# lebrice/blurred-GAN

Measured on AMD Instinct MI355X. Metric: images/sec (G+D+GP step), higher is better.
Workload: dtype f32; 1 GPU; celeba64 64x64x3 batch 256/GPU, blur sigma 5.0 (31 taps), D-step+GP+G-step+Adam; global_batch=256, parallelism=dp1

## Files before the change

### blurred-gan_amd/csrc/conv_wgrad.hip

```cpp
#include "conv_common.h"
#include <algorithm>
#include <cmath>
#include <cstdlib>
#include <mutex>
#include <type_traits>
#include <utility>

namespace {

typedef float floatx16 __attribute__((ext_vector_type(16)));

struct WgradParams {
  const float* X;
  const float* DY;
  float* out;
  int B, H, W, Ci, Ho, Wo, Co;
  int k, s, pt, pl;
  int M;
  int chunk;
  int ksplit;
  int tiles_m, tiles_n, xcd_swizzle;
  float beta, scale;
  unsigned x_bytes, dy_bytes;
  unsigned mul_hw, sh_hw, mul_w, sh_w;
// ... 988 lines not shown
    }
  };

  int strip = blockIdx.x;
  prefetch(strip);
  stash(0);
  __syncthreads();
  int buf = 0;
  for (; strip < nstrips; strip += gridDim.x, buf ^= 1) {
#pragma unroll
    for (int ks = 0; ks < KSW; ++ks) { bc[ks][0] = bn[ks][0]; bc[ks][1] = bn[ks][1]; }
    prefetch(strip + gridDim.x);
    const float* xb = c16_lds + buf * kC16Rows * RS + (2 * r) * RS + (half * (WO / 2) + kq + 1) * 16 + li;
#pragma unroll
    for (int ks = 0; ks < KSW; ++ks)
#pragma unroll
      for (int kh = 0; kh < 5; ++kh)
#pragma unroll
        for (int kw = 0; kw < 5; ++kw) {
          const int par = (kw + 1) & 1, fl = kw == 0 ? -1 : (kw - 1) / 2;
          const float a = xb[kh * RS + par * PS + (4 * ks + fl) * 16];
          acc[kh * 5 + kw][0] = __builtin_amdgcn_mfma_f32_16x16x4f32(a, bc[ks][0], acc[kh * 5 + kw][0], 0, 0, 0);
          acc[kh * 5 + kw][1] = __builtin_amdgcn_mfma_f32_16x16x4f32(a, bc[ks][1], acc[kh * 5 + kw][1], 0, 0, 0);
        }
    stash(buf ^ 1);
    __syncthreads();
  }
  float* red = c16_lds;
  for (int w = 0; w < 4; ++w) {
    __syncthreads();
    if (wave == w) {
#pragma unroll
      for (int t = 0; t < 25; ++t)
#pragma unroll
        for (int nt = 0; nt < 2; ++nt)
#pragma unroll
          for (int rr = 0; rr < 4; ++rr) {
            float* q = red + ((t * 2 + nt) * 4 + rr) * 64 + lane;
            *q = (w == 0 ? 0.f : *q) + acc[t][nt][rr];
          }
    }
  }
  __syncthreads();
  float* out = p.out + (size_t)blockIdx.x * 25 * 16 * 32;
  for (int e = tid; e < 25 * 2 * 4 * 64; e += 256) {
    const int l = e & 63, slot = e >> 6;
    const int rr = slot & 3, nt = (slot >> 2) & 1, t = slot >> 3;
    out[(size_t)(t * 16 + 4 * (l >> 4) + rr) * 32 + nt * 16 + (l & 15)] = red[e];
  }
}

template <int LGWO>
struct StripGeom {
  static constexpr int WO = 1 << LGWO, W = 2 * WO, R = 64 / WO, RX = 2 * R + 3, WP = W + 3;
  static constexpr int XROW = WP * 32, XBUF = RX * XROW, YBUF = 64 * 64, BUF = XBUF + YBUF;
  static constexpr int NX = RX * W * 8, NLX = (NX + 255) / 256, NL = NLX + 4;
  static constexpr size_t lds_bytes = (size_t)2 * BUF * sizeof(float);
};

typedef float floatx2 __attribute__((ext_vector_type(2)));

template <int O0>
__device__ inline void strip_read2(floatx2& dst, unsigned addr) {
  asm volatile("ds_read2st64_b32 %0, %1 offset0:%2 offset1:%3" : "=v"(dst) : "v"(addr), "n"(O0), "n"(O0 + 2));
}
__device__ inline void strip_mfma(floatx16& acc, float a, float b) {
  asm volatile("v_mfma_f32_32x32x2_f32 %0, %1, %2, %0" : "+a"(acc) : "v"(a), "v"(b));
}
template <int LGWO, int Q, int T>
__device__ inline void strip_fetch(floatx2 (&af)[13], floatx2& bf, const unsigned (&aaddr)[13], unsigned baddr) {
  constexpr int WO = 1 << LGWO, WP = 2 * WO + 3, pix = 4 * Q, oyl = pix >> LGWO, ox = pix & (WO - 1);
  if constexpr (T < 13) strip_read2<oyl * WP + ox>(af[T], aaddr[T]);
  else strip_read2<pix>(bf, baddr);
}
typedef float floatx4v __attribute__((ext_vector_type(4)));
__device__ inline void strip_gload(floatx4v& dst, unsigned off, __amdgpu_buffer_rsrc_t rs) {
  asm volatile("buffer_load_dwordx4 %0, %1, %2, 0 offen" : "=v"(dst) : "v"(off), "s"(rs));
}
template <int VM>
__device__ inline void strip_lwrite(unsigned addr, const floatx4v& v) {
  asm volatile("s_waitcnt vmcnt(%2)\n\tds_write_b128 %0, %1" : : "v"(addr), "v"(v), "n"(VM) : "memory");
}
template <int NL_, int PPP_>
struct StripPieces {
  static constexpr int NL = NL_, PPP = PPP_, LAG = 3;
  floatx4v pf[NL_];
  unsigned off[NL_];
  unsigned dst[NL_];
  __amdgpu_buffer_rsrc_t rsX, rsY;
  int nlx;
};
template <int LGWO, int Q, int I, class PC>
__device__ inline void strip_steps(floatx16 (&acc)[13], floatx2 (&af)[2][13], floatx2 (&bf)[2], const unsigned (&aaddr)[13], unsigned baddr,
                                   bool mine, PC& pc) {
  if constexpr (I < 26) {
    constexpr int C = Q & 1, H = I / 13, T = I % 13;
    if (T < 12 || mine) {
      if constexpr (H == 0) strip_mfma(acc[T], af[C][T].x, bf[C].x);
      else strip_mfma(acc[T], af[C][T].y, bf[C].y);
    }
    if constexpr (Q + 1 < 16 && I <= 13) strip_fetch<LGWO, Q + 1, I>(af[C ^ 1], bf[C ^ 1], aaddr, baddr);
    constexpr int P = PC::PPP, NL = PC::NL, LAG = PC::LAG;
    if constexpr (I >= 14 && I <= 18 && ((I - 14) & 1) == 0) {
      constexpr int u = (I - 14) / 2, l = Q * P + u;
      if constexpr (u < P && l < NL) {
        if (l < pc.nlx) strip_gload(pc.pf[l], pc.off[l], pc.rsX);
        else strip_gload(pc.pf[l], pc.off[l], pc.rsY);
      }
    }
    if constexpr (I >= 19 && I <= 23 && ((I - 19) & 1) == 0) {
      constexpr int u = (I - 19) / 2, lw = (Q - LAG) * P + u;
      if constexpr (Q >= LAG && u < P && lw < NL) {
        constexpr int issued = (Q + 1) * P < NL ? (Q + 1) * P : NL;
        strip_lwrite<issued - lw - 1>(pc.dst[lw], pc.pf[lw]);
      }
    }
    strip_steps<LGWO, Q, I + 1>(acc, af, bf, aaddr, baddr, mine, pc);
  }
}
template <int LGWO, int T>
__device__ inline void strip_fetch_first(floatx2 (&af)[2][13], floatx2 (&bf)[2], const unsigned (&aaddr)[13], unsigned baddr) {
  if constexpr (T <= 13) {
    strip_fetch<LGWO, 0, T>(af[0], bf[0], aaddr, baddr);
    strip_fetch_first<LGWO, T + 1>(af, bf, aaddr, baddr);
  }
}
template <int LGWO, int Q, class PC>
__device__ inline void strip_pairs(floatx16 (&acc)[13], floatx2 (&af)[2][13], floatx2 (&bf)[2], const unsigned (&aaddr)[13], unsigned baddr,
                                   PC& pc, int th) {
  if constexpr (Q < 16) {
    asm volatile("s_waitcnt lgkmcnt(0)" ::: "memory");
    strip_steps<LGWO, Q, 0>(acc, af, bf, aaddr, baddr, (Q & 1) == th, pc);
    strip_pairs<LGWO, Q + 1>(acc, af, bf, aaddr, baddr, pc, th);
  }
}

template <int LGWO>
__global__ __launch_bounds__(256, 1) void conv_wgrad_strip_kernel(const WgradParams p, int nstrips, int strips_per_img, int strips_per_wg,
                                                                   int ntile) {
  using G = StripGeom<LGWO>;
  constexpr int WO = G::WO, W = G::W, R = G::R, RX = G::RX, WP = G::WP, XROW = G::XROW, XBUF = G::XBUF, BUF = G::BUF;
  constexpr int NLX = G::NLX, NL = G::NL, NT = 13;
  constexpr unsigned kOob = 0x80000000u;
  extern __shared__ __attribute__((aligned(16))) float strip_lds[];
  const int tid = threadIdx.x, lane = tid & 63, wave = __builtin_amdgcn_readfirstlane(tid >> 6);
  const int th = wave >> 1, nh = wave & 1;
  int tile, z;
  {
    const int idx = blockIdx.x;
    if ((p.ksplit & 7) == 0) {
      const int j = idx >> 3;
      tile = j % ntile;
      z = (idx & 7) + 8 * (j / ntile);
    } else {
      tile = idx % ntile;
      z = idx / ntile;
    }
  }
  const int tile_m = tile / p.tiles_n, tile_n = tile - tile_m * p.tiles_n;
  const int ci0 = tile_m * 32, co0 = tile_n * 64;
  const __amdgpu_buffer_rsrc_t rsX = __builtin_amdgcn_make_buffer_rsrc(const_cast<float*>(p.X), 0, (int)p.x_bytes, 0x00020000);
  const __amdgpu_buffer_rsrc_t rsY = __builtin_amdgcn_make_buffer_rsrc(const_cast<float*>(p.DY), 0, (int)p.dy_bytes, 0x00020000);

  for (int i = tid; i < 2 * RX * 3 * 32; i += 256) {
    const int e = i & 31, rest = i >> 5, c = rest % 3, row = rest / 3;
    const int bufi = row / RX, rr = row - bufi * RX;
    strip_lds[bufi * BUF + rr * XROW + (c == 0 ? 0 : (W + c)) * 32 + e] = 0.f;
  }

  floatx16 acc[NT];
#pragma unroll
  for (int t = 0; t < NT; ++t)
#pragma unroll
    for (int r = 0; r < 16; ++r) acc[t][r] = 0.f;

  constexpr int NP = 16, LAG = 3, PPP = (NL + NP - LAG - 1) / (NP - LAG) > 2 ? (NL + NP - LAG - 1) / (NP - LAG) : 2;
  static_assert(PPP <= 3 && PPP * (NP - LAG) >= NL, "every piece of the next strip must be requested and written within one strip");
  StripPieces<NL, PPP> pc;
  pc.rsX = rsX; pc.rsY = rsY; pc.nlx = NLX;
  int x_rr[NLX], x_dst[NLX];
  unsigned x_off[NLX];
#pragma unroll
  for (int l = 0; l < NLX; ++l) {
    const int item = l * 256 + tid;
    const int rr = item / (W * 8), rem = item - rr * (W * 8);
    const int xc = rem >> 3, q = rem & 7;
    x_rr[l] = item < G::NX ? rr : 1 << 20;
    x_dst[l] = item < G::NX ? rr * XROW + (xc + 1) * 32 + q * 4 : (tid & 7) * 4;
    x_off[l] = (unsigned)(((rr * W + xc) * p.Ci + ci0 + q * 4) * 4);
  }
  const int y_dst = XBUF + (tid >> 4) * 64 + (tid & 15) * 4;
  const unsigned y_off = (unsigned)(((tid >> 4) * p.Co + co0 + (tid & 15) * 4) * 4);

  const int s_begin = z * strips_per_wg, s_end = min(nstrips, s_begin + strips_per_wg);
  auto plan = [&](int sidx, int buf) {
    const bool live = sidx < s_end;
    const int b = sidx / strips_per_img, oy0 = (sidx - b * strips_per_img) * R;
    const unsigned xbase = (unsigned)(((b * p.H + 2 * oy0 - 1) * W) * p.Ci * 4);
    const unsigned ybase = (unsigned)(((b * p.Ho + oy0) * WO) * p.Co * 4);
#pragma unroll
    for (int l = 0; l < NL; ++l) {
      if (l < NLX) {
        const int y = 2 * oy0 - 1 + x_rr[l];
        const bool ok = live && (unsigned)y < (unsigned)p.H;
        pc.off[l] = ok ? xbase + x_off[l] : kOob;
        pc.dst[l] = (unsigned)((buf * BUF + x_dst[l]) * 4);
      } else {
        pc.off[l] = live ? ybase + (unsigned)((l - NLX) * 16 * p.Co * 4) + y_off : kOob;
        pc.dst[l] = (unsigned)((buf * BUF + y_dst + (l - NLX) * 16 * 64) * 4);
      }
    }
  };

  plan(s_begin, 0);
#pragma unroll
  for (int l = 0; l < NL; ++l) {
    if (l < NLX) strip_gload(pc.pf[l], pc.off[l], rsX);
    else strip_gload(pc.pf[l], pc.off[l], rsY);
  }
#pragma unroll
  for (int l = 0; l < NL; ++l) {
    if (l == 0) strip_lwrite<0>(pc.dst[l], pc.pf[l]);
    else asm volatile("ds_write_b128 %0, %1" : : "v"(pc.dst[l]), "v"(pc.pf[l]) : "memory");
  }
  asm volatile("s_waitcnt lgkmcnt(0)" ::: "memory");
  __syncthreads();

  const int kk = lane >> 5, li = lane & 31;
  int a_tap[NT];
#pragma unroll
  for (int t = 0; t < NT; ++t) {
    const int tap = t < 12 ? th * 13 + t : 12;
    const int kh = tap / 5, kw = tap - kh * 5;
    a_tap[t] = (kh * WP + kw) * 32 + kk * 64 + li;
  }
  const int b_base = XBUF + kk * 64 + nh * 32 + li;

  int buf = 0;
  for (int sidx = s_begin; sidx < s_end; ++sidx, buf ^= 1) {
    unsigned aaddr[NT];
#pragma unroll
    for (int t = 0; t < NT; ++t) aaddr[t] = (unsigned)((buf * BUF + a_tap[t]) * 4);
    const unsigned baddr = (unsigned)((buf * BUF + b_base) * 4);
    floatx2 af[2][NT], bf[2];
    plan(sidx + 1, buf ^ 1);
    asm volatile("" ::: "memory");
    strip_fetch_first<LGWO, 0>(af, bf, aaddr, baddr);
    strip_pairs<LGWO, 0>(acc, af, bf, aaddr, baddr, pc, th);
    asm volatile("s_waitcnt lgkmcnt(0)" ::: "memory");
    __syncthreads();
  }

  if (th == 1) {
#pragma unroll
    for (int r = 0; r < 16; ++r) strip_lds[(nh * 16 + r) * 64 + lane] = acc[12][r];
  }
  __syncthreads();
  if (th == 0) {
#pragma unroll
    for (int r = 0; r < 16; ++r) acc[12][r] += strip_lds[(nh * 16 + r) * 64 + lane];
  }
  float* out = p.out + (size_t)z * 25 * p.Ci * p.Co;
#pragma unroll
  for (int t = 0; t < NT; ++t) {
    const int tap = t < 12 ? th * 13 + t : 12;
    if (t < 12 || th == 0) {
      float* o = out + (size_t)tap * p.Ci * p.Co + (size_t)ci0 * p.Co + co0 + nh * 32 + li;
#pragma unroll
      for (int r = 0; r < 16; ++r) o[(size_t)((r & 3) + 8 * (r >> 2) + 4 * kk) * p.Co] = acc[t][r];
    }
  }
}

__global__ __launch_bounds__(256) void wgrad_reduce_kernel(const float* __restrict__ slabs, float* __restrict__ dw, int n,
                                                           int ksplit, float beta, float scale) {
  __shared__ float4 red[4][64];
  const int lane = threadIdx.x & 63, zg = threadIdx.x >> 6;
  const int e = (blockIdx.x * 64 + lane) * 4;
  float4 s = make_float4(0.f, 0.f, 0.f, 0.f);
  if (e < n) {
    int z = zg;
    for (; z + 12 < ksplit; z += 16) {
      float4 v[4];
#pragma unroll
      for (int i = 0; i < 4; ++i) v[i] = *reinterpret_cast<const float4*>(slabs + (size_t)(z + 4 * i) * n + e);
#pragma unroll
      for (int i = 0; i < 4; ++i) { s.x += v[i].x; s.y += v[i].y; s.z += v[i].z; s.w += v[i].w; }
    }
    {
      float4 v[4];
#pragma unroll
      for (int i = 0; i < 4; ++i)
        v[i] = z + 4 * i < ksplit ? *reinterpret_cast<const float4*>(slabs + (size_t)(z + 4 * i) * n + e) : make_float4(0.f, 0.f, 0.f, 0.f);
#pragma unroll
      for (int i = 0; i < 4; ++i)
        if (z + 4 * i < ksplit) { s.x += v[i].x; s.y += v[i].y; s.z += v[i].z; s.w += v[i].w; }
    }
  }
  red[zg][lane] = s;
  __syncthreads();
  if (zg != 0 || e >= n) return;
  const float4 a = red[0][lane], b = red[1][lane], c = red[2][lane], d = red[3][lane];
  float4 o = make_float4(scale * ((a.x + b.x) + (c.x + d.x)), scale * ((a.y + b.y) + (c.y + d.y)),
                         scale * ((a.z + b.z) + (c.z + d.z)), scale * ((a.w + b.w) + (c.w + d.w)));
  if (beta != 0.f) {
    const float4 q = *reinterpret_cast<const float4*>(dw + e);
    o.x += beta * q.x; o.y += beta * q.y; o.z += beta * q.z; o.w += beta * q.w;
  }
  *reinterpret_cast<float4*>(dw + e) = o;
}

__global__ __launch_bounds__(1024) void wgrad_reduce_tall_kernel(const float* __restrict__ slabs, float* __restrict__ dw, int n,
                                                                 int ksplit, float beta, float scale) {
  __shared__ float4 red[64][16];
  const int c = threadIdx.x & 15, zg = threadIdx.x >> 4;
  const int e = (blockIdx.x * 16 + c) * 4;
  float4 s0 = make_float4(0.f, 0.f, 0.f, 0.f), s1 = s0;
  if (e < n) {
    int z = zg;
    for (; z + 64 < ksplit; z += 128) {
      const float4 v0 = *reinterpret_cast<const float4*>(slabs + (size_t)z * n + e);
      const float4 v1 = *reinterpret_cast<const float4*>(slabs + (size_t)(z + 64) * n + e);
      s0.x += v0.x; s0.y += v0.y; s0.z += v0.z; s0.w += v0.w;
      s1.x += v1.x; s1.y += v1.y; s1.z += v1.z; s1.w += v1.w;
    }
    if (z < ksplit) {
      const float4 v0 = *reinterpret_cast<const float4*>(slabs + (size_t)z * n + e);
      s0.x += v0.x; s0.y += v0.y; s0.z += v0.z; s0.w += v0.w;
    }
  }
  red[zg][c] = make_float4(s0.x + s1.x, s0.y + s1.y, s0.z + s1.z, s0.w + s1.w);
  __syncthreads();
  for (int h = 32; h > 0; h >>= 1) {
    if (zg < h) {
      const float4 a = red[zg][c], b = red[zg + h][c];
      red[zg][c] = make_float4(a.x + b.x, a.y + b.y, a.z + b.z, a.w + b.w);
    }
    __syncthreads();
  }
  if (zg != 0 || e >= n) return;
  const float4 a = red[0][c];
  float4 o = make_float4(scale * a.x, scale * a.y, scale * a.z, scale * a.w);
  if (beta != 0.f) {
    const float4 q = *reinterpret_cast<const float4*>(dw + e);
    o.x += beta * q.x; o.y += beta * q.y; o.z += beta * q.z; o.w += beta * q.w;
  }
  *reinterpret_cast<float4*>(dw + e) = o;
}

__global__ __launch_bounds__(256) void wgrad_reduce_scalar_kernel(const float* __restrict__ slabs, float* __restrict__ dw, int n,
                                                                  int ksplit, float beta, float scale) {
  const int e = blockIdx.x * 256 + threadIdx.x;
  if (e >= n) return;
  float s = 0.f;
  for (int z = 0; z < ksplit; ++z) s += slabs[(size_t)z * n + e];
  dw[e] = (beta != 0.f ? beta * dw[e] : 0.f) + scale * s;
}

struct WgradPlan {
  int mode;
  int ksplit, chunk, tiles_m, tiles_n, bkp, taps_in_grid;
  int always_slab;
};

inline bool strip_ok(int H, int W, int Ci, int Co, int k, int s) {
  if (k != 5 || s != 2 || (H & 1) || (W & 1) || Ci % 32 || Co % 64) return false;
  const int Wo = W / 2, Ho = H / 2;
  if (Wo != 8 && Wo != 16 && Wo != 32) return false;
  return Ho % (64 / Wo) == 0;
}

WgradPlan plan_wgrad(int B, int H, int W, int Ci, int Co, int k, int s) {
  WgradPlan pl{};
  int Ho, Wo, pt, pp;
  bg::same_pads(H, k, s, &Ho, &pt);
  bg::same_pads(W, k, s, &Wo, &pp);
  const long M = (long)B * Ho * Wo;
  const bool mfma = (Ci % 4 == 0) && (Co % 4 == 0) && Ci >= 16 && Co >= 16;
  const int kk = k * k;
  const bool thin_ci = Ci <= 4 && Co % 4 == 0 && Co >= 16 && kk * Ci <= 128;
  const bool thin_co = Co <= 4 && Ci % 4 == 0 && Ci >= 16 && s == 1 && kk * Co <= 128;
  int bm = 0, bn = 0;
  if (!mfma && !thin_ci && !thin_co) {
    pl.mode = 0;
    const long nblk = bg::cdiv((size_t)k * k * Ci * Co, 256);
    long want = std::max(1L, 2048 / nblk);
    long chunk = std::max(256L, (M + want - 1) / want);
    pl.chunk = (int)chunk;
    pl.ksplit = (int)((M + chunk - 1) / chunk);
    return pl;
  }
  if (strip_ok(H, W, Ci, Co, k, s) && !getenv("BG_WGRAD_NO_STRIP")) {
    pl.mode = 33;
    pl.bkp = 2;
    pl.tiles_m = Ci / 32;
    pl.tiles_n = Co / 64;
    const long nstrips = (long)B * (Ho / (64 / Wo));
    const long ntile = (long)pl.tiles_m * pl.tiles_n;
    long ks = std::max(1L, std::min(nstrips, std::max(1L, 256 / ntile)));
    long spw = (nstrips + ks - 1) / ks;
    ks = (nstrips + spw - 1) / spw;
    pl.ksplit = (int)ks;
    pl.chunk = (int)spw;
    pl.taps_in_grid = 0;
    pl.always_slab = 1;
    return pl;
  }
  if (Ci == 16 && Co == 32 && k == 5 && s == 2 && !(H & 1) && !(W & 1) && (Wo == 32 || Wo == 64) && !(Ho & 1) && !getenv("BG_NO_C16")) {
    pl.mode = 32;
    pl.bkp = 4;
    const long nstrips = (long)B * (Ho / 2);
    pl.ksplit = (int)std::max<long>(2, std::min<long>(nstrips, 256));
    pl.chunk = (int)nstrips;
    pl.tiles_m = pl.tiles_n = 1;
    pl.taps_in_grid = 0;
    return pl;
  }
  if (thin_ci && k * Ci <= 16 && (k == 5 || k == 3) && (Co == 16 || Co == 32 || Co == 64) && Wo % 4 == 0 && !getenv("BG_WGRAD_NO_TC")) {
    pl.mode = 31;
    pl.bkp = 4;
    const int rb = s == 2 ? 8 : 16;
    const long nblocks = (long)B * bg::cdiv(Ho, rb);
    pl.ksplit = (int)std::max<long>(2, std::min<long>(nblocks, 1024));
    pl.chunk = (int)nblocks;
    pl.tiles_m = pl.tiles_n = 1;
    pl.taps_in_grid = 0;
    return pl;
  }
  if (thin_ci) {
    const int gw = kk * Ci <= 32 ? 32 : (kk * Ci <= 96 ? 96 : 128);
    pl.bkp = 64;
    if (gw == 32) { pl.mode = 10; bm = 32; bn = 64; }
    else if (gw == 96) { pl.mode = 11; bm = 96; bn = 32; }
    else { pl.mode = 12; bm = 128; bn = 32; }
    pl.tiles_m = 1;
    pl.tiles_n = bg::cdiv(Co, bn);
    pl.taps_in_grid = 0;
  } else if (thin_co && (Ci == 16 || Ci == 32) && (k == 5 || k == 3) && k * Co <= 16 && W % 4 == 0 && !getenv("BG_WGRAD_NO_TC")) {
    pl.mode = 30;
    pl.bkp = 4;
    const long nblocks = (long)B * bg::cdiv(H, kTcRows);
    pl.ksplit = (int)std::max<long>(2, std::min<long>(nblocks, 1024));
    pl.chunk = (int)nblocks;
    pl.tiles_m = pl.tiles_n = 1;
    pl.taps_in_grid = 0;
    return pl;
  } else if (thin_co) {
    const int gw = kk * Co <= 32 ? 32 : (kk * Co <= 96 ? 96 : 128);
    pl.bkp = 64;
    if (gw == 32) { pl.mode = 20; bm = 64; bn = 32; }
// ... 93 lines not shown
    auto magic = [](unsigned d, unsigned* mul, unsigned* sh) {
      unsigned sft = 0;
      while ((1ull << sft) < d) ++sft;
      *mul = (unsigned)((1ull << (31 + sft)) / d + 1);
      *sh = 31 + sft;
    };
    magic((unsigned)(p.Ho * p.Wo), &p.mul_hw, &p.sh_hw);
    magic((unsigned)p.Wo, &p.mul_w, &p.sh_w);
    auto lg2 = [](int v) { int l = 0; while ((1 << l) < v) ++l; return l; };
    p.lg_w = lg2(p.Wo); p.lg_h = lg2(p.Ho);
    p.pow2 = ((1 << p.lg_w) == p.Wo && (1 << p.lg_h) == p.Ho) ? 1 : 0;
    p.lg_b = lg2(B);
    static const int no_pm = getenv("BG_NO_POS_MAJOR") ? 1 : 0;
    static const int pm_pow2 = getenv("BG_WGRAD_PM_POW2") ? 1 : 0;
    const bool b_ok = pm_pow2 ? (1 << p.lg_b) == B : B % 128 == 0;
    if (p.pow2 && !no_pm && b_ok && B >= 128 && p.Ho * p.Wo <= 16) p.pow2 = 2;
    p.x_bytes = (unsigned)((size_t)B * H * W * Cin * sizeof(float));
    p.dy_bytes = (unsigned)((size_t)p.M * Cout * sizeof(float));
  }
  p.chunk = pl.chunk; p.ksplit = pl.ksplit; p.tiles_n = pl.tiles_n; p.tiles_m = pl.tiles_m;
  {
    static const int swz = getenv("BG_WGRAD_SWZ") ? atoi(getenv("BG_WGRAD_SWZ")) : 0;
    static const int swz_tg = getenv("BG_WGRAD_SWZ_TG") ? atoi(getenv("BG_WGRAD_SWZ_TG")) : 1;
    p.xcd_swizzle = (pl.mode == 6 || pl.mode == 7) ? swz_tg : swz;
  }
  p.beta = beta; p.scale = scale;
  p.order_n = 0;
  {
    static const int no_sort = getenv("BG_NO_TILE_SORT") ? 1 : 0;
    if (p.pow2 == 2 && pl.taps_in_grid == 1 && pl.mode >= 1 && pl.mode <= 5 && !no_sort && ksize * ksize <= 32) {
      int live[32], idx[32];
      for (int t = 0; t < ksize * ksize; ++t) {
        const int dyk = t / ksize - p.pt, dxk = t % ksize - p.pl;
        auto floordiv = [](int a, int b) { return a >= 0 ? a / b : -((-a + b - 1) / b); };
        const int oh_lo = std::max(0, (-dyk + stride - 1) / stride), oh_hi = std::min(p.Ho - 1, floordiv(H - 1 - dyk, stride));
        const int ow_lo = std::max(0, (-dxk + stride - 1) / stride), ow_hi = std::min(p.Wo - 1, floordiv(W - 1 - dxk, stride));
        live[t] = std::max(0, oh_hi - oh_lo + 1) * std::max(0, ow_hi - ow_lo + 1);
        idx[t] = t;
      }
      std::stable_sort(idx, idx + ksize * ksize, [&](int a, int b) { return live[a] > live[b]; });
      for (int t = 0; t < ksize * ksize; ++t) p.tap_order[t] = (unsigned char)idx[t];
      p.order_n = ksize * ksize;
    }
  }
  p.out = slabs ? static_cast<float*>(ws_d) : dw;
  const double flops = 2.0 * p.M * (double)nout;
  const double abytes = 4.0 * ((double)B * H * W * Cin + (double)p.M * Cout + (double)nout * (beta != 0.f ? 2 : 1));
  int rc;
  if (pl.mode == 0) {
    bg::Launch L(stream, "conv_wgrad_direct", flops, abytes);
    bg::launch(wgrad_direct_kernel, dim3(bg::cdiv(nout, 256), pl.ksplit), dim3(256), 0, L.s, p);
    rc = L.done("wgrad_direct_kernel");
  } else if (pl.mode == 33) {
    bg::Launch L(stream, "conv_wgrad_mfma", flops, abytes);
    const int lgwo = p.Wo == 32 ? 5 : (p.Wo == 16 ? 4 : 3);
    const int spi = p.Ho / (64 / p.Wo), nstrips = B * spi, ntile = pl.tiles_m * pl.tiles_n;
    BG_LDS_ATTR_ONCE_V(conv_wgrad_strip_kernel<5>, StripGeom<5>::lds_bytes);
    BG_LDS_ATTR_ONCE_V(conv_wgrad_strip_kernel<4>, StripGeom<4>::lds_bytes);
    BG_LDS_ATTR_ONCE_V(conv_wgrad_strip_kernel<3>, StripGeom<3>::lds_bytes);
    const dim3 grid((unsigned)(ntile * pl.ksplit));
    if (lgwo == 5) bg::launch((conv_wgrad_strip_kernel<5>), grid, dim3(256), StripGeom<5>::lds_bytes, L.s, p, nstrips, spi, pl.chunk, ntile);
    else if (lgwo == 4) bg::launch((conv_wgrad_strip_kernel<4>), grid, dim3(256), StripGeom<4>::lds_bytes, L.s, p, nstrips, spi, pl.chunk, ntile);
    else bg::launch((conv_wgrad_strip_kernel<3>), grid, dim3(256), StripGeom<3>::lds_bytes, L.s, p, nstrips, spi, pl.chunk, ntile);
    rc = L.done("conv_wgrad_strip_kernel");
  } else if (pl.mode == 32) {
    bg::Launch L(stream, "conv_wgrad_c16", flops, abytes);
    const int spi = p.Ho / 2, nstrips = B * spi;
    const size_t lds = std::max((size_t)2 * kC16Rows * 2 * (p.Wo + 2) * 16, (size_t)25 * 2 * 4 * 64) * sizeof(float);
    BG_LDS_ATTR_ONCE_V(conv_wgrad_c16_kernel<64>, 150 * 1024);
    BG_LDS_ATTR_ONCE_V(conv_wgrad_c16_kernel<32>, 150 * 1024);
    if (p.Wo == 64) bg::launch((conv_wgrad_c16_kernel<64>), dim3(pl.ksplit), dim3(256), lds, L.s, p, nstrips, spi);
    else bg::launch((conv_wgrad_c16_kernel<32>), dim3(pl.ksplit), dim3(256), lds, L.s, p, nstrips, spi);
    rc = L.done("conv_wgrad_c16_kernel");
  } else if (pl.mode == 31) {
    bg::Launch L(stream, "conv_wgrad_mfma_thin_ci", flops, abytes);
    const int rb = stride == 2 ? 8 : 16;
    const int bpi = (int)bg::cdiv(p.Ho, rb), nblocks = B * bpi;
    const int nt = Cout / 16;
    const size_t lds = std::max((size_t)((rb - 1) * stride + ksize) * (W * Cin + 2 * kTiHalo), (size_t)ksize * nt * 4 * 64) * sizeof(float);
    BG_REQUIRE(lds <= 64 * 1024, BG_ERR_UNSUPPORTED, "bg_conv2d_bwd_filter: thin-Ci row kernel needs %zu bytes of LDS", lds);
#define BG_TI(NTv, Kv) bg::launch((conv_wgrad_thin_ci_kernel<NTv, Kv>), dim3(pl.ksplit), dim3(256), lds, L.s, p, nblocks, bpi, rb)
    if (ksize == 5) { if (nt == 1) BG_TI(1, 5); else if (nt == 2) BG_TI(2, 5); else BG_TI(4, 5); }
    else { if (nt == 1) BG_TI(1, 3); else if (nt == 2) BG_TI(2, 3); else BG_TI(4, 3); }
#undef BG_TI
    rc = L.done("conv_wgrad_thin_ci_kernel");
  } else if (pl.mode == 30) {
    bg::Launch L(stream, "conv_wgrad_mfma_thin_co", flops, abytes);
    const int bpi = (int)bg::cdiv(H, kTcRows), nblocks = B * bpi;
    const int mt = Cin / 16;
    const size_t lds = std::max((size_t)(kTcRows + ksize - 1) * (W * Cout + 2 * kTcHalo), (size_t)4 * ksize * mt * 4 * 64) * sizeof(float);
    BG_REQUIRE(lds <= 64 * 1024, BG_ERR_UNSUPPORTED, "bg_conv2d_bwd_filter: thin-Co row kernel needs %zu bytes of LDS", lds);
    if (ksize == 5 && mt == 2) bg::launch((conv_wgrad_thin_co_kernel<2, 5>), dim3(pl.ksplit), dim3(256), lds, L.s, p, nblocks, bpi);
    else if (ksize == 5) bg::launch((conv_wgrad_thin_co_kernel<1, 5>), dim3(pl.ksplit), dim3(256), lds, L.s, p, nblocks, bpi);
    else if (mt == 2) bg::launch((conv_wgrad_thin_co_kernel<2, 3>), dim3(pl.ksplit), dim3(256), lds, L.s, p, nblocks, bpi);
    else bg::launch((conv_wgrad_thin_co_kernel<1, 3>), dim3(pl.ksplit), dim3(256), lds, L.s, p, nblocks, bpi);
    rc = L.done("conv_wgrad_thin_co_kernel");
  } else {
    dim3 grid(pl.tiles_m * pl.tiles_n, pl.taps_in_grid == 1 ? ksize * ksize : (pl.taps_in_grid == 2 ? ksize : 1), pl.ksplit);
    bg::Launch L(stream, pl.mode >= 20 ? "conv_wgrad_mfma_thin_co" : (pl.mode >= 10 ? "conv_wgrad_mfma_thin_ci" : "conv_wgrad_mfma"), flops, abytes);
    const dim3 grid1((unsigned)(grid.x * grid.y * grid.z));
    switch (pl.mode) {
#define BG_V3(BMv, BNv, BKv, WMv, WNv, WKv)                                                                               \
  do {                                                                                                                   \
    if (p.pow2 == 2) bg::launch((conv_wgrad_v3_kernel<BMv, BNv, BKv, WMv, WNv, WKv, 2>), grid1, dim3(256), 0, L.s, p);     \
    else if (p.pow2 == 1) bg::launch((conv_wgrad_v3_kernel<BMv, BNv, BKv, WMv, WNv, WKv, 1>), grid1, dim3(256), 0, L.s, p); \
    else bg::launch((conv_wgrad_v3_kernel<BMv, BNv, BKv, WMv, WNv, WKv, 0>), grid1, dim3(256), 0, L.s, p);        \
  } while (0)
      case 1: BG_V3(128, 128, 32, 2, 2, 1); break;
      case 2: BG_V3(64, 64, 32, 2, 2, 1); break;
      case 3: BG_V3(64, 32, 64, 2, 1, 2); break;
      case 4: BG_V3(32, 64, 64, 1, 2, 2); break;
      case 5: BG_V3(32, 32, 128, 1, 1, 4); break;
#undef BG_V3
      case 6: bg::launch((conv_wgrad_tg_kernel<5, 64, 2, 2>), grid1, dim3(256), 0, L.s, p); break;
      case 7: bg::launch((conv_wgrad_tg_kernel<5, 32, 1, 4>), grid1, dim3(256), 0, L.s, p); break;
      case 10: bg::launch((conv_wgrad_kernel<32, 64, 64, 1, 2, 2, 1>), grid, dim3(256), 0, L.s, p); break;
// ... 27 lines not shown
```

Measured before the change: 32500 images/s.

## Skip padding-only MFMAs in wgrad strip kernel and add multi-image 4x4 strips

Adds a compile-time plan that, when a strip covers a whole 8x8 output image, tells which filter taps and pixel pairs touch only zero padding. It then drops those MFMAs and LDS reads and rebalances taps across the two wave halves by live work. It also adds an opt-in multi-image strip variant for 4x4 outputs that packs several padded images into one LDS buffer. The cost is more template instantiations and code complexity. The 4x4 path is gated behind an environment variable, so only the 8x8 skip path runs by default.

```diff
diff --git a/blurred-gan_amd/csrc/conv_wgrad.hip b/blurred-gan_amd/csrc/conv_wgrad.hip
--- a/blurred-gan_amd/csrc/conv_wgrad.hip
+++ b/blurred-gan_amd/csrc/conv_wgrad.hip
@@ -1064,26 +1064,107 @@
 
 template <int LGWO>
 struct StripGeom {
-  static constexpr int WO = 1 << LGWO, W = 2 * WO, R = 64 / WO, RX = 2 * R + 3, WP = W + 3;
+  static constexpr bool MULTI = LGWO == 2;
+  static constexpr int WO = 1 << LGWO, W = 2 * WO, R = 64 / WO, WP = W + 3;
+  static constexpr int NI = MULTI ? 64 / (WO * WO) : 1, IMR = W + 2;
+  static constexpr int RX = MULTI ? NI * IMR + 1 : 2 * R + 3;
   static constexpr int XROW = WP * 32, XBUF = RX * XROW, YBUF = 64 * 64, BUF = XBUF + YBUF;
-  static constexpr int NX = RX * W * 8, NLX = (NX + 255) / 256, NL = NLX + 4;
+  static constexpr int NXR = MULTI ? NI * W : RX;
+  static constexpr int NX = NXR * W * 8, NLX = (NX + 255) / 256, NL = NLX + 4;
   static constexpr size_t lds_bytes = (size_t)2 * BUF * sizeof(float);
+  static constexpr int IMG_U = IMR * WP / 2;
+  static constexpr int XKK = MULTI ? IMG_U : 1, XH = MULTI ? 2 * IMG_U : 2;
+  static constexpr int YKK = MULTI ? WO * WO : 1, YH = MULTI ? 2 * WO * WO : 2;
+  static constexpr int xo(int Q) { return MULTI ? (Q >> LGWO) * WP + (Q & (WO - 1)) : ((4 * Q) >> LGWO) * WP + ((4 * Q) & (WO - 1)); }
+  static constexpr int yo(int Q) { return MULTI ? Q : 4 * Q; }
+  static_assert(!MULTI || (IMR * WP) % 2 == 0, "image stride must be whole 64-float units");
+  static_assert(xo(15) + XH <= 255 && yo(15) + YH <= 255, "ds_read2st64 offsets are 8 bits");
 };
 
+template <int LGWO, bool WHOLE>
+struct StripPlan {
+  bool live[25][16][2] = {};
+  unsigned char tap[2][13] = {};
+  bool share[2][16][2] = {};
+  static constexpr bool pix_live(int kh, int kw, int oy, int ox, int H) {
+    return 2 * oy + kh - 1 >= 0 && 2 * oy + kh - 1 < H && 2 * ox + kw - 1 >= 0 && 2 * ox + kw - 1 < H;
+  }
+  constexpr StripPlan() {
+    constexpr int WO = 1 << LGWO, H = 2 * WO;
+    int n[25] = {};
+    for (int t = 0; t < 25; ++t)
+      for (int Q = 0; Q < 16; ++Q)
+        for (int h = 0; h < 2; ++h) {
+          bool l = true;
+          if (WHOLE && LGWO == 2) l = pix_live(t / 5, t % 5, Q >> 2, Q & 3, H);
+          if (WHOLE && LGWO == 3) {
+            const int p0 = 4 * Q + 2 * h;
+            l = pix_live(t / 5, t % 5, p0 >> 3, p0 & 7, H) || pix_live(t / 5, t % 5, (p0 + 1) >> 3, (p0 + 1) & 7, H);
+          }
+          live[t][Q][h] = l;
+          n[t] += l;
+        }
+    tap[0][12] = tap[1][12] = 12;
+    for (int Q = 0; Q < 16; ++Q)
+      for (int h = 0; h < 2; ++h) { share[0][Q][h] = (Q & 1) == 0; share[1][Q][h] = (Q & 1) == 1; }
+    if (!WHOLE) {
+      for (int t = 0; t < 12; ++t) { tap[0][t] = t; tap[1][t] = 13 + t; }
+      return;
+    }
+    int order[24] = {};
+    for (int t = 0, i = 0; t < 25; ++t)
+      if (t != 12) order[i++] = t;
+    for (int i = 1; i < 24; ++i) {
+      const int v = order[i];
+      int j = i;
+      while (j > 0 && n[order[j - 1]] < n[v]) { order[j] = order[j - 1]; --j; }
+      order[j] = v;
+    }
+    int s[2] = {0, 0}, c[2] = {0, 0};
+    for (int i = 0; i < 24; ++i) {
+      const int t = order[i];
+      const int hf = (c[0] < 12 && (c[1] == 12 || s[0] <= s[1])) ? 0 : 1;
+      tap[hf][c[hf]++] = (unsigned char)t;
+      s[hf] += n[t];
+    }
+  }
+  constexpr bool runs(int th, int Q, int h, int T, bool skip) const {
+    return (T < 12 || share[th][Q][h]) && (!skip || live[tap[th][T]][Q][h]);
+  }
+  constexpr int mfmas(bool skip) const {
+    int n = 0;
+    for (int th = 0; th < 2; ++th)
+      for (int Q = 0; Q < 16; ++Q)
+        for (int h = 0; h < 2; ++h)
+          for (int T = 0; T < 13; ++T) n += runs(th, Q, h, T, skip);
+    return n;
+  }
+  constexpr bool reads(int th, int Q, int T, bool skip) const {
+    if (T < 13) return runs(th, Q, 0, T, skip) || runs(th, Q, 1, T, skip);
+    for (int u = 0; u < 13; ++u)
+      if (reads(th, Q, u, skip)) return true;
+    return false;
+  }
+};
+template <int LGWO, bool WHOLE>
+struct StripPlanOf {
+  static constexpr StripPlan<LGWO, WHOLE> v{};
+};
+
 typedef float floatx2 __attribute__((ext_vector_type(2)));
 
-template <int O0>
+template <int O0, int O1>
 __device__ inline void strip_read2(floatx2& dst, unsigned addr) {
-  asm volatile("ds_read2st64_b32 %0, %1 offset0:%2 offset1:%3" : "=v"(dst) : "v"(addr), "n"(O0), "n"(O0 + 2));
+  asm volatile("ds_read2st64_b32 %0, %1 offset0:%2 offset1:%3" : "=v"(dst) : "v"(addr), "n"(O0), "n"(O1));
 }
 __device__ inline void strip_mfma(floatx16& acc, float a, float b) {
   asm volatile("v_mfma_f32_32x32x2_f32 %0, %1, %2, %0" : "+a"(acc) : "v"(a), "v"(b));
 }
 template <int LGWO, int Q, int T>
 __device__ inline void strip_fetch(floatx2 (&af)[13], floatx2& bf, const unsigned (&aaddr)[13], unsigned baddr) {
-  constexpr int WO = 1 << LGWO, WP = 2 * WO + 3, pix = 4 * Q, oyl = pix >> LGWO, ox = pix & (WO - 1);
-  if constexpr (T < 13) strip_read2<oyl * WP + ox>(af[T], aaddr[T]);
-  else strip_read2<pix>(bf, baddr);
+  using G = StripGeom<LGWO>;
+  if constexpr (T < 13) strip_read2<G::xo(Q), G::xo(Q) + G::XH>(af[T], aaddr[T]);
+  else strip_read2<G::yo(Q), G::yo(Q) + G::YH>(bf, baddr);
 }
 typedef float floatx4v __attribute__((ext_vector_type(4)));
 __device__ inline void strip_gload(floatx4v& dst, unsigned off, __amdgpu_buffer_rsrc_t rs) {
@@ -1102,57 +1183,68 @@
   __amdgpu_buffer_rsrc_t rsX, rsY;
   int nlx;
 };
-template <int LGWO, int Q, int I, class PC>
+template <int LGWO, bool WHOLE, bool SKIP, int TH, int Q, int I, class PC>
 __device__ inline void strip_steps(floatx16 (&acc)[13], floatx2 (&af)[2][13], floatx2 (&bf)[2], const unsigned (&aaddr)[13], unsigned baddr,
                                    bool mine, PC& pc) {
   if constexpr (I < 26) {
     constexpr int C = Q & 1, H = I / 13, T = I % 13;
-    if (T < 12 || mine) {
+    constexpr auto& P = StripPlanOf<LGWO, WHOLE>::v;
+    if constexpr (TH < 0) {
+      if (T < 12 || mine) {
+        if constexpr (H == 0) strip_mfma(acc[T], af[C][T].x, bf[C].x);
+        else strip_mfma(acc[T], af[C][T].y, bf[C].y);
+      }
+    } else if constexpr (P.runs(TH, Q, H, T, SKIP)) {
       if constexpr (H == 0) strip_mfma(acc[T], af[C][T].x, bf[C].x);
       else strip_mfma(acc[T], af[C][T].y, bf[C].y);
     }
-    if constexpr (Q + 1 < 16 && I <= 13) strip_fetch<LGWO, Q + 1, I>(af[C ^ 1], bf[C ^ 1], aaddr, baddr);
-    constexpr int P = PC::PPP, NL = PC::NL, LAG = PC::LAG;
+    if constexpr (Q + 1 < 16 && I <= 13) {
+      if constexpr (TH < 0) strip_fetch<LGWO, Q + 1, I>(af[C ^ 1], bf[C ^ 1], aaddr, baddr);
+      else if constexpr (P.reads(TH, Q + 1, I, SKIP)) strip_fetch<LGWO, Q + 1, I>(af[C ^ 1], bf[C ^ 1], aaddr, baddr);
+    }
+    constexpr int PP = PC::PPP, NL = PC::NL, LAG = PC::LAG;
     if constexpr (I >= 14 && I <= 18 && ((I - 14) & 1) == 0) {
-      constexpr int u = (I - 14) / 2, l = Q * P + u;
-      if constexpr (u < P && l < NL) {
+      constexpr int u = (I - 14) / 2, l = Q * PP + u;
+      if constexpr (u < PP && l < NL) {
         if (l < pc.nlx) strip_gload(pc.pf[l], pc.off[l], pc.rsX);
         else strip_gload(pc.pf[l], pc.off[l], pc.rsY);
       }
     }
     if constexpr (I >= 19 && I <= 23 && ((I - 19) & 1) == 0) {
-      constexpr int u = (I - 19) / 2, lw = (Q - LAG) * P + u;
-      if constexpr (Q >= LAG && u < P && lw < NL) {
-        constexpr int issued = (Q + 1) * P < NL ? (Q + 1) * P : NL;
+      constexpr int u = (I - 19) / 2, lw = (Q - LAG) * PP + u;
+      if constexpr (Q >= LAG && u < PP && lw < NL) {
+        constexpr int issued = (Q + 1) * PP < NL ? (Q + 1) * PP : NL;
         strip_lwrite<issued - lw - 1>(pc.dst[lw], pc.pf[lw]);
       }
     }
-    strip_steps<LGWO, Q, I + 1>(acc, af, bf, aaddr, baddr, mine, pc);
-  }
-}
-template <int LGWO, int T>
+    strip_steps<LGWO, WHOLE, SKIP, TH, Q, I + 1>(acc, af, bf, aaddr, baddr, mine, pc);
+  }
+}
+template <int LGWO, bool WHOLE, bool SKIP, int TH, int T>
 __device__ inline void strip_fetch_first(floatx2 (&af)[2][13], floatx2 (&bf)[2], const unsigned (&aaddr)[13], unsigned baddr) {
   if constexpr (T <= 13) {
-    strip_fetch<LGWO, 0, T>(af[0], bf[0], aaddr, baddr);
-    strip_fetch_first<LGWO, T + 1>(af, bf, aaddr, baddr);
-  }
-}
-template <int LGWO, int Q, class PC>
+    if constexpr (TH < 0) strip_fetch<LGWO, 0, T>(af[0], bf[0], aaddr, baddr);
+    else if constexpr (StripPlanOf<LGWO, WHOLE>::v.reads(TH, 0, T, SKIP)) strip_fetch<LGWO, 0, T>(af[0], bf[0], aaddr, baddr);
+    strip_fetch_first<LGWO, WHOLE, SKIP, TH, T + 1>(af, bf, aaddr, baddr);
+  }
+}
+template <int LGWO, bool WHOLE, bool SKIP, int TH, int Q, class PC>
 __device__ inline void strip_pairs(floatx16 (&acc)[13], floatx2 (&af)[2][13], floatx2 (&bf)[2], const unsigned (&aaddr)[13], unsigned baddr,
                                    PC& pc, int th) {
   if constexpr (Q < 16) {
     asm volatile("s_waitcnt lgkmcnt(0)" ::: "memory");
-    strip_steps<LGWO, Q, 0>(acc, af, bf, aaddr, baddr, (Q & 1) == th, pc);
-    strip_pairs<LGWO, Q + 1>(acc, af, bf, aaddr, baddr, pc, th);
-  }
-}
-
-template <int LGWO>
+    strip_steps<LGWO, WHOLE, SKIP, TH, Q, 0>(acc, af, bf, aaddr, baddr, (Q & 1) == th, pc);
+    strip_pairs<LGWO, WHOLE, SKIP, TH, Q + 1>(acc, af, bf, aaddr, baddr, pc, th);
+  }
+}
+
+template <int LGWO, bool WHOLE, bool SKIP>
 __global__ __launch_bounds__(256, 1) void conv_wgrad_strip_kernel(const WgradParams p, int nstrips, int strips_per_img, int strips_per_wg,
                                                                    int ntile) {
   using G = StripGeom<LGWO>;
   constexpr int WO = G::WO, W = G::W, R = G::R, RX = G::RX, WP = G::WP, XROW = G::XROW, XBUF = G::XBUF, BUF = G::BUF;
   constexpr int NLX = G::NLX, NL = G::NL, NT = 13;
+  static_assert(!G::MULTI || WHOLE, "multi-image strips are whole images");
   constexpr unsigned kOob = 0x80000000u;
   extern __shared__ __attribute__((aligned(16))) float strip_lds[];
   const int tid = threadIdx.x, lane = tid & 63, wave = __builtin_amdgcn_readfirstlane(tid >> 6);
@@ -1174,17 +1266,20 @@
   const __amdgpu_buffer_rsrc_t rsX = __builtin_amdgcn_make_buffer_rsrc(const_cast<float*>(p.X), 0, (int)p.x_bytes, 0x00020000);
   const __amdgpu_buffer_rsrc_t rsY = __builtin_amdgcn_make_buffer_rsrc(const_cast<float*>(p.DY), 0, (int)p.dy_bytes, 0x00020000);
 
-  for (int i = tid; i < 2 * RX * 3 * 32; i += 256) {
-    const int e = i & 31, rest = i >> 5, c = rest % 3, row = rest / 3;
-    const int bufi = row / RX, rr = row - bufi * RX;
-    strip_lds[bufi * BUF + rr * XROW + (c == 0 ? 0 : (W + c)) * 32 + e] = 0.f;
-  }
-
-  floatx16 acc[NT];
-#pragma unroll
-  for (int t = 0; t < NT; ++t)
-#pragma unroll
-    for (int r = 0; r < 16; ++r) acc[t][r] = 0.f;
+  if constexpr (G::MULTI) {
+    for (int i = tid; i < 2 * RX * WP * 8; i += 256) {
+      const int q = i & 7, rest = i >> 3, c = rest % WP, row = rest / WP;
+      const int bufi = row / RX, rr = row - bufi * RX, y = rr % G::IMR;
+      if (c == 0 || c > W || y == 0 || y > W)
+        *reinterpret_cast<float4*>(strip_lds + bufi * BUF + rr * XROW + c * 32 + q * 4) = make_float4(0.f, 0.f, 0.f, 0.f);
+    }
+  } else {
+    for (int i = tid; i < 2 * RX * 3 * 32; i += 256) {
+      const int e = i & 31, rest = i >> 5, c = rest % 3, row = rest / 3;
+      const int bufi = row / RX, rr = row - bufi * RX;
+      strip_lds[bufi * BUF + rr * XROW + (c == 0 ? 0 : (W + c)) * 32 + e] = 0.f;
+    }
+  }
 
   constexpr int NP = 16, LAG = 3, PPP = (NL + NP - LAG - 1) / (NP - LAG) > 2 ? (NL + NP - LAG - 1) / (NP - LAG) : 2;
   static_assert(PPP <= 3 && PPP * (NP - LAG) >= NL, "every piece of the next strip must be requested and written within one strip");
@@ -1197,8 +1292,9 @@
     const int item = l * 256 + tid;
     const int rr = item / (W * 8), rem = item - rr * (W * 8);
     const int xc = rem >> 3, q = rem & 7;
+    const int lrow = G::MULTI ? (rr / W) * G::IMR + rr % W + 1 : rr;
     x_rr[l] = item < G::NX ? rr : 1 << 20;
-    x_dst[l] = item < G::NX ? rr * XROW + (xc + 1) * 32 + q * 4 : (tid & 7) * 4;
+    x_dst[l] = item < G::NX ? lrow * XROW + (xc + 1) * 32 + q * 4 : (tid & 7) * 4;
     x_off[l] = (unsigned)(((rr * W + xc) * p.Ci + ci0 + q * 4) * 4);
   }
   const int y_dst = XBUF + (tid >> 4) * 64 + (tid & 15) * 4;
@@ -1207,14 +1303,13 @@
   const int s_begin = z * strips_per_wg, s_end = min(nstrips, s_begin + strips_per_wg);
   auto plan = [&](int sidx, int buf) {
     const bool live = sidx < s_end;
-    const int b = sidx / strips_per_img, oy0 = (sidx - b * strips_per_img) * R;
-    const unsigned xbase = (unsigned)(((b * p.H + 2 * oy0 - 1) * W) * p.Ci * 4);
+    const int b = G::MULTI ? sidx * G::NI : sidx / strips_per_img, oy0 = G::MULTI ? 0 : (sidx - b * strips_per_img) * R;
+    const unsigned xbase = G::MULTI ? (unsigned)(b * p.H * W * p.Ci * 4) : (unsigned)(((b * p.H + 2 * oy0 - 1) * W) * p.Ci * 4);
     const unsigned ybase = (unsigned)(((b * p.Ho + oy0) * WO) * p.Co * 4);
 #pragma unroll
     for (int l = 0; l < NL; ++l) {
       if (l < NLX) {
-        const int y = 2 * oy0 - 1 + x_rr[l];
-        const bool ok = live && (unsigned)y < (unsigned)p.H;
+        const bool ok = G::MULTI ? live && x_rr[l] < G::NXR : live && (unsigned)(2 * oy0 - 1 + x_rr[l]) < (unsigned)p.H;
         pc.off[l] = ok ? xbase + x_off[l] : kOob;
         pc.dst[l] = (unsigned)((buf * BUF + x_dst[l]) * 4);
       } else {
@@ -1238,50 +1333,62 @@
   asm volatile("s_waitcnt lgkmcnt(0)" ::: "memory");
   __syncthreads();
 
-  const int kk = lane >> 5, li = lane & 31;
-  int a_tap[NT];
-#pragma unroll
-  for (int t = 0; t < NT; ++t) {
-    const int tap = t < 12 ? th * 13 + t : 12;
-    const int kh = tap / 5, kw = tap - kh * 5;
-    a_tap[t] = (kh * WP + kw) * 32 + kk * 64 + li;
-  }
-  const int b_base = XBUF + kk * 64 + nh * 32 + li;
-
-  int buf = 0;
-  for (int sidx = s_begin; sidx < s_end; ++sidx, buf ^= 1) {
-    unsigned aaddr[NT];
-#pragma unroll
-    for (int t = 0; t < NT; ++t) aaddr[t] = (unsigned)((buf * BUF + a_tap[t]) * 4);
-    const unsigned baddr = (unsigned)((buf * BUF + b_base) * 4);
-    floatx2 af[2][NT], bf[2];
-    plan(sidx + 1, buf ^ 1);
-    asm volatile("" ::: "memory");
-    strip_fetch_first<LGWO, 0>(af, bf, aaddr, baddr);
-    strip_pairs<LGWO, 0>(acc, af, bf, aaddr, baddr, pc, th);
-    asm volatile("s_waitcnt lgkmcnt(0)" ::: "memory");
+  auto run = [&](auto th_c) {
+    constexpr int TH = decltype(th_c)::value;
+    constexpr auto& P = StripPlanOf<LGWO, WHOLE>::v;
+    floatx16 acc[NT];
+#pragma unroll
+    for (int t = 0; t < NT; ++t)
+#pragma unroll
+      for (int r = 0; r < 16; ++r) acc[t][r] = 0.f;
+    const int kk = lane >> 5, li = lane & 31;
+    int a_tap[NT], a_tapn[NT];
+#pragma unroll
+    for (int t = 0; t < NT; ++t) {
+      const int tap = TH >= 0 ? P.tap[TH < 0 ? 0 : TH][t] : (th ? P.tap[1][t] : P.tap[0][t]);
+      const int kh = tap / 5, kw = tap - kh * 5;
+      a_tapn[t] = tap;
+      a_tap[t] = (kh * WP + kw) * 32 + kk * G::XKK * 64 + li;
+    }
+    const int b_base = XBUF + kk * G::YKK * 64 + nh * 32 + li;
+    int buf = 0;
+    for (int sidx = s_begin; sidx < s_end; ++sidx, buf ^= 1) {
+      unsigned aaddr[NT];
+#pragma unroll
+      for (int t = 0; t < NT; ++t) aaddr[t] = (unsigned)((buf * BUF + a_tap[t]) * 4);
+      const unsigned baddr = (unsigned)((buf * BUF + b_base) * 4);
+      floatx2 af[2][NT], bf[2];
+      plan(sidx + 1, buf ^ 1);
+      asm volatile("" ::: "memory");
+      strip_fetch_first<LGWO, WHOLE, SKIP, TH, 0>(af, bf, aaddr, baddr);
+      strip_pairs<LGWO, WHOLE, SKIP, TH, 0>(acc, af, bf, aaddr, baddr, pc, th);
+      asm volatile("s_waitcnt lgkmcnt(0)" ::: "memory");
+      __syncthreads();
+    }
+
+    const bool first = TH >= 0 ? TH == 0 : th == 0;
+    if (!first) {
+#pragma unroll
+      for (int r = 0; r < 16; ++r) strip_lds[(nh * 16 + r) * 64 + lane] = acc[12][r];
+    }
     __syncthreads();
-  }
-
-  if (th == 1) {
-#pragma unroll
-    for (int r = 0; r < 16; ++r) strip_lds[(nh * 16 + r) * 64 + lane] = acc[12][r];
-  }
-  __syncthreads();
-  if (th == 0) {
-#pragma unroll
-    for (int r = 0; r < 16; ++r) acc[12][r] += strip_lds[(nh * 16 + r) * 64 + lane];
-  }
-  float* out = p.out + (size_t)z * 25 * p.Ci * p.Co;
-#pragma unroll
-  for (int t = 0; t < NT; ++t) {
-    const int tap = t < 12 ? th * 13 + t : 12;
-    if (t < 12 || th == 0) {
-      float* o = out + (size_t)tap * p.Ci * p.Co + (size_t)ci0 * p.Co + co0 + nh * 32 + li;
-#pragma unroll
-      for (int r = 0; r < 16; ++r) o[(size_t)((r & 3) + 8 * (r >> 2) + 4 * kk) * p.Co] = acc[t][r];
-    }
-  }
+    if (first) {
+#pragma unroll
+      for (int r = 0; r < 16; ++r) acc[12][r] += strip_lds[(nh * 16 + r) * 64 + lane];
+    }
+    float* out = p.out + (size_t)z * 25 * p.Ci * p.Co;
+#pragma unroll
+    for (int t = 0; t < NT; ++t) {
+      if (t < 12 || first) {
+        float* o = out + (size_t)a_tapn[t] * p.Ci * p.Co + (size_t)ci0 * p.Co + co0 + nh * 32 + li;
+#pragma unroll
+        for (int r = 0; r < 16; ++r) o[(size_t)((r & 3) + 8 * (r >> 2) + 4 * kk) * p.Co] = acc[t][r];
+      }
+    }
+  };
+  if constexpr (!WHOLE) run(std::integral_constant<int, -1>{});
+  else if (th == 0) run(std::integral_constant<int, 0>{});
+  else run(std::integral_constant<int, 1>{});
 }
 
 __global__ __launch_bounds__(256) void wgrad_reduce_kernel(const float* __restrict__ slabs, float* __restrict__ dw, int n,
@@ -1375,9 +1482,13 @@
   int always_slab;
 };
 
-inline bool strip_ok(int H, int W, int Ci, int Co, int k, int s) {
+inline bool strip_ok(int B, int H, int W, int Ci, int Co, int k, int s) {
   if (k != 5 || s != 2 || (H & 1) || (W & 1) || Ci % 32 || Co % 64) return false;
   const int Wo = W / 2, Ho = H / 2;
+  if (Wo == 4) {
+    const char* e = getenv("BG_WGRAD_STRIP4");
+    return Ho == 4 && B % StripGeom<2>::NI == 0 && e && atoi(e) == 1;
+  }
   if (Wo != 8 && Wo != 16 && Wo != 32) return false;
   return Ho % (64 / Wo) == 0;
 }
@@ -1402,12 +1513,12 @@
     pl.ksplit = (int)((M + chunk - 1) / chunk);
     return pl;
   }
-  if (strip_ok(H, W, Ci, Co, k, s) && !getenv("BG_WGRAD_NO_STRIP")) {
+  if (strip_ok(B, H, W, Ci, Co, k, s) && !getenv("BG_WGRAD_NO_STRIP")) {
     pl.mode = 33;
     pl.bkp = 2;
     pl.tiles_m = Ci / 32;
     pl.tiles_n = Co / 64;
-    const long nstrips = (long)B * (Ho / (64 / Wo));
+    const long nstrips = Wo == 4 ? (long)B / StripGeom<2>::NI : (long)B * (Ho / (64 / Wo));
     const long ntile = (long)pl.tiles_m * pl.tiles_n;
     long ks = std::max(1L, std::min(nstrips, std::max(1L, 256 / ntile)));
     long spw = (nstrips + ks - 1) / ks;
@@ -1607,16 +1718,27 @@
     bg::launch(wgrad_direct_kernel, dim3(bg::cdiv(nout, 256), pl.ksplit), dim3(256), 0, L.s, p);
     rc = L.done("wgrad_direct_kernel");
   } else if (pl.mode == 33) {
-    bg::Launch L(stream, "conv_wgrad_mfma", flops, abytes);
-    const int lgwo = p.Wo == 32 ? 5 : (p.Wo == 16 ? 4 : 3);
-    const int spi = p.Ho / (64 / p.Wo), nstrips = B * spi, ntile = pl.tiles_m * pl.tiles_n;
-    BG_LDS_ATTR_ONCE_V(conv_wgrad_strip_kernel<5>, StripGeom<5>::lds_bytes);
-    BG_LDS_ATTR_ONCE_V(conv_wgrad_strip_kernel<4>, StripGeom<4>::lds_bytes);
-    BG_LDS_ATTR_ONCE_V(conv_wgrad_strip_kernel<3>, StripGeom<3>::lds_bytes);
+    bg::Launch L(stream, "conv_wgrad_strip", flops, abytes);
+    const int lgwo = p.Wo == 32 ? 5 : (p.Wo == 16 ? 4 : (p.Wo == 8 ? 3 : 2));
+    const int spi = lgwo == 2 ? 1 : p.Ho / (64 / p.Wo), nstrips = lgwo == 2 ? B / StripGeom<2>::NI : B * spi, ntile = pl.tiles_m * pl.tiles_n;
+    const bool skip = !getenv("BG_WGRAD_STRIP_NO_SKIP"), whole = lgwo == 2 || (lgwo == 3 && p.Ho == 8 && skip);
+    BG_LDS_ATTR_ONCE_V((conv_wgrad_strip_kernel<5, false, false>), StripGeom<5>::lds_bytes);
+    BG_LDS_ATTR_ONCE_V((conv_wgrad_strip_kernel<4, false, false>), StripGeom<4>::lds_bytes);
+    BG_LDS_ATTR_ONCE_V((conv_wgrad_strip_kernel<3, false, false>), StripGeom<3>::lds_bytes);
+    BG_LDS_ATTR_ONCE_V((conv_wgrad_strip_kernel<3, true, true>), StripGeom<3>::lds_bytes);
+    BG_LDS_ATTR_ONCE_V((conv_wgrad_strip_kernel<2, true, true>), StripGeom<2>::lds_bytes);
+    BG_LDS_ATTR_ONCE_V((conv_wgrad_strip_kernel<2, true, false>), StripGeom<2>::lds_bytes);
+    if (L.prof && whole && skip)
+      L.exec_flops(flops * (lgwo == 3 ? StripPlanOf<3, true>::v.mfmas(true) : StripPlanOf<2, true>::v.mfmas(true)) / 800.0);
     const dim3 grid((unsigned)(ntile * pl.ksplit));
-    if (lgwo == 5) bg::launch((conv_wgrad_strip_kernel<5>), grid, dim3(256), StripGeom<5>::lds_bytes, L.s, p, nstrips, spi, pl.chunk, ntile);
-    else if (lgwo == 4) bg::launch((conv_wgrad_strip_kernel<4>), grid, dim3(256), StripGeom<4>::lds_bytes, L.s, p, nstrips, spi, pl.chunk, ntile);
-    else bg::launch((conv_wgrad_strip_kernel<3>), grid, dim3(256), StripGeom<3>::lds_bytes, L.s, p, nstrips, spi, pl.chunk, ntile);
+#define BG_STRIP(LG, WH, SK) bg::launch((conv_wgrad_strip_kernel<LG, WH, SK>), grid, dim3(256), StripGeom<LG>::lds_bytes, L.s, p, nstrips, spi, pl.chunk, ntile)
+    if (lgwo == 5) BG_STRIP(5, false, false);
+    else if (lgwo == 4) BG_STRIP(4, false, false);
+    else if (lgwo == 3 && !whole) BG_STRIP(3, false, false);
+    else if (lgwo == 3) BG_STRIP(3, true, true);
+    else if (skip) BG_STRIP(2, true, true);
+    else BG_STRIP(2, true, false);
+#undef BG_STRIP
     rc = L.done("conv_wgrad_strip_kernel");
   } else if (pl.mode == 32) {
     bg::Launch L(stream, "conv_wgrad_c16", flops, abytes);
```

After: 32540 images/s (median of 4 runs). About the same (+0.1%).
